# POSTECH-CVLab/InstaOrder

Hardware: AMD Instinct MI355X
Metric: instance-pairs/sec (fwd+bwd) (higher is better)
Workload: dtype f32; 1 GPU; InstaOrderNet_o, pair-batch 256 per GPU at 256x256x5, fp32, fwd+bwd+SGD (BASELINE.json configs[1]); inputs=resident in HBM, pairs_per_gpu=256, input_size=256, parallelism=dp1, hip_graph=True, setup_steps=0, inputs_distinct=True

## Files before the change

### include/instaorder_hip.h

```cpp
#ifndef INSTAORDER_HIP_H
#define INSTAORDER_HIP_H

#include <stddef.h>
#include <stdint.h>

#ifdef __cplusplus
extern "C" {
#endif

#define IO_OK 0
#define IO_ERR_SHAPE (-1)
#define IO_ERR_WORKSPACE (-2)
#define IO_ERR_LAUNCH (-3)
#define IO_ERR_STATE (-4)
#define IO_ERR_NODEVICE (-5)

#if !defined(__HIP__) && !defined(HIP_INCLUDE_HIP_HIP_RUNTIME_API_H)
typedef void* hipStream_t;
#endif

int io_abi_version(void);
const char* io_last_error_string(void);
int io_device_count(void);
int io_set_winograd(int on);
// ... 207 lines not shown
                             const float* scale, const float* shift, float* dgamma, float* dbeta, void* dyb,
                             float* workspace, size_t workspace_floats, int dtype, int gw, hipStream_t stream);
size_t io_stem_packed_floats(int real_channels);
size_t io_stem_wgrad_exact_workspace_bytes(int N, int H, int W, int real_channels);
int io_stem_fwd_bnstats_exact(const float* x8, const float* w, float* y, int N, int H, int W, int real_channels, int G,
                              const float* gamma, const float* beta, float* running_mean, float* running_var,
                              float momentum, float eps, float* mean, float* rstd, float* scale, float* shift,
                              float* workspace, size_t workspace_floats, float* packed, hipStream_t stream);
int io_stem_wgrad_exact(const float* x8, const float* dy, float* dw, int N, int H, int W, int real_channels,
                        void* workspace, size_t workspace_bytes, float* packed, hipStream_t stream);
int io_stem_wgrad_exact_bn(const float* x8, const float* da, const float* y, float* dw, int N, int H, int W,
                           int real_channels, int G, const float* gamma, const float* mean, const float* rstd,
                           const float* scale, const float* shift, float* dgamma, float* dbeta, float* coef,
                           float* bn_partial, size_t bn_partial_floats, void* workspace, size_t workspace_bytes,
                           float* packed, hipStream_t stream);

size_t io_bn_tile_partial_floats(int M, int C, int G);
int io_bn_bwd_coefs_dt(const void* dz, const void* y, int M, int C, int G, const float* gamma, const float* mean,
                       const float* rstd, float* dgamma, float* dbeta, float* coef, float* partial,
                       size_t partial_floats, int dtype, hipStream_t stream);
int io_bn_bwd_coefs_from_tile_partials(float* p1, float* p2, int M, int C, int G, const float* gamma, const float* mean,
                                       const float* rstd, float* dgamma, float* dbeta, float* coef, hipStream_t stream);
typedef struct io_dgrad_fused {
    const void* xb_y;
    const float* xb_coef;
    void* xb_dy_out;
    const void* add;
    const void* relu_mask;
    const void* ep_y;
    const float *ep_mean, *ep_rstd, *ep_scale, *ep_shift;
// ... 159 lines not shown
```

### instaorder_amd/_lib.py

```python
import ctypes as C
import os

_HERE = os.path.dirname(os.path.abspath(__file__))
LIB_PATH = os.environ.get("IO_LIB_PATH") or os.path.join(_HERE, "libinstaorder_hip.so")
_lib = None

c_float_p = C.c_void_p


def csrc_digest():
    import glob
    import hashlib
    h = hashlib.sha256()
    files = sorted(glob.glob(os.path.join(_HERE, "csrc", "*.hip")) + glob.glob(os.path.join(_HERE, "csrc", "*.h")))
    files.append(os.path.join(os.path.dirname(_HERE), "include", "instaorder_hip.h"))
    for f in files:
        h.update(os.path.basename(f).encode())
        h.update(open(f, "rb").read())
    return h.hexdigest()[:16]


class TensorInfo(C.Structure):
    _fields_ = [("name", C.c_char * 64), ("kind", C.c_int), ("ndim", C.c_int), ("shape", C.c_long * 4),
                ("offset", C.c_long), ("numel_storage", C.c_long), ("cin_storage", C.c_int),
# ... 140 lines not shown
    "io_add": (_I, [_P, _P, _Z, _P, _I, _P]),
    "io_colsum_partial_floats": (_Z, [_I, _I]),
    "io_colsum": (_I, [_P, _I, _I, _P, _P, _Z, _I, _P]),
    "io_head1_fwd": (_I, [_P, _I, _I, _I, _P, _P, _I, _P, _I, _P]),
    "io_head1_bwd": (_I, [_P, _P, _P, _I, _I, _I, _P, _I, _P, _P, _P, _P, _Z, _I, _P]),
    "io_conv2d_fwd_bnstats_dt": (_I, [_P, _P, _P, _I, _I, _I, _I, _I, _I, _I, _I, _I, _I, _P, _P, _P, _P, _F, _F, _P,
                                      _P, _P, _P, _P, _Z, _I, _I, _P]),
    "io_conv2d_fwd_bias_dt": (_I, [_P, _P, _P, _I, _I, _I, _I, _I, _I, _I, _I, _I, _P, _P, _I, _I, _I, _P]),
    "io_stem_packed_floats": (_Z, [_I]),
    "io_stem_wgrad_exact_workspace_bytes": (_Z, [_I, _I, _I, _I]),
    "io_stem_fwd_bnstats_exact": (_I, [_P, _P, _P, _I, _I, _I, _I, _I, _P, _P, _P, _P, _F, _F, _P, _P, _P, _P, _P, _Z, _P,
                                       _P]),
    "io_stem_wgrad_exact": (_I, [_P, _P, _P, _I, _I, _I, _I, _P, _Z, _P, _P]),
    "io_stem_wgrad_exact_bn": (_I, [_P, _P, _P, _P, _I, _I, _I, _I, _I, _P, _P, _P, _P, _P, _P, _P, _P, _P, _Z, _P, _Z, _P,
                                    _P]),
    "io_stem_wgrad_bn_bf16": (_I, [_P, _P, _P, _P, _I, _I, _I, _I, _P, _P, _P, _P, _P, _P, _P, _P, _P, _Z, _P, _Z, _P]),
    "io_stem_wgrad_bf16_workspace_bytes": (_Z, []),
    "io_debug_last_wgrad_route": (_I, []),
    "io_conv2d_fwd_resid": (_I, [_P, _P, _P, _P, _P, _I, _I, _I, _I, _I, _I, _P, _P, _P, _P, _P, _P, _P, _F, _F, _P, _P, _P,
                                 _P, _P, _Z, _P]),
    "io_smooth_loss_workspace_floats": (_Z, [_I, _I, _I]),
    "io_smooth_loss_fwd": (_I, [_P, _P, _I, _I, _I, _F, _P, _P, _P, _Z, _P]),
    "io_smooth_loss_bwd": (_I, [_P, _P, _P, _F, _I, _I, _I, _I, _P, _P]),
    "io_disp_order_workspace_floats": (_Z, [_I, _I, _I]),
    "io_disp_order_count": (_I, [_P, _P, _P, _P, _P, _P, _I, _I, _I, _I, _F, _P, _P, _Z, _P]),
    "io_bn_tile_partial_floats": (_Z, [_I, _I, _I]),
    "io_bn_bwd_coefs_dt": (_I, [_P, _P, _I, _I, _I, _P, _P, _P, _P, _P, _P, _P, _Z, _I, _P]),
    "io_bn_bwd_coefs_from_tile_partials": (_I, [_P, _P, _I, _I, _I, _P, _P, _P, _P, _P, _P, _P]),
    "io_conv2d_dgrad_fused_dt": (_I, [_P, _P, _P, _I, _I, _I, _I, _I, _I, _I, _I, _I, C.POINTER(DgradFused), _I, _P]),
    "io_conv2d_dgrad_bnbwd_dt": (_I, [_P, _P, _P, _I, _I, _I, _I, _I, _I, _I, _I, _P, _I, _P, _P, _P, _P, _P, _P, _P, _P, _P,
# ... 62 lines not shown
```

### instaorder_amd/csrc/bn.hip

```cpp
#include "io_common.h"

namespace {

constexpr int kThreads = 256;

template <typename T> __device__ __forceinline__ f32x4 ld4(const T* p) { return io_ldv(p); }
template <typename T> __device__ __forceinline__ void st4(T* p, f32x4 v) { io_stv(p, v); }

__device__ __forceinline__ f32x4 bn_affine(f32x4 y, f32x4 mean, f32x4 scale, f32x4 shift) {
    f32x4 r;
#pragma unroll
    for (int k = 0; k < 4; ++k) r[k] = __builtin_fmaf(y[k] - mean[k], scale[k], shift[k]);
    return r;
}

template <typename T> struct Chunk {
    static constexpr int VEC = 16 / (int)sizeof(T), NV = VEC / 4;
    f32x4 v[NV];
};
__device__ __forceinline__ Chunk<float> ldc(const float* p) {
    Chunk<float> c;
    c.v[0] = *reinterpret_cast<const f32x4*>(p);
    return c;
}
// ... 323 lines not shown
                            }
                            s1[i][k] += dd;
                            s2[i][k] += dd * ((yv[u].v[k] - mu[i].v[k]) * rs[i].v[k]);
                        }
                    }
                }
            }
        }
    }
    const size_t o = ((size_t)g * nb + b) * C;
#pragma unroll
    for (int k = 0; k < NV; ++k) {
        f32x4 t1[2] = {s1[0][k], s1[1][k]}, t2[2] = {s2[0][k], s2[1][k]};
        reduce_rows_store<2>(cm, t1, t2, p1 + o + 4 * k, p2 + o + 4 * k, CV, VEC);
    }
}

__global__ __launch_bounds__(256) void bn_bwd_finalize_kernel(const float* __restrict__ p1,
                                                             const float* __restrict__ p2, int nb, int G, int Mg,
                                                             int C, float* __restrict__ dgamma,
                                                             float* __restrict__ dbeta, float* __restrict__ c1,
                                                             float* __restrict__ c2,
                                                             const float* __restrict__ xgamma = nullptr,
                                                             const float* __restrict__ xmean = nullptr,
                                                             const float* __restrict__ xrstd = nullptr,
                                                             float* __restrict__ c3 = nullptr) {
    constexpr int U = 16;
    __shared__ double sh[2][32][8];
    const int tx = threadIdx.x & 7, ty = threadIdx.x >> 3;
    const int c = blockIdx.x * 8 + tx;
// ... 452 lines not shown
    const int rpb = bn_rows_per_block(Mg, G, &nb);
    float* p1 = partial;
    float* p2 = partial + (size_t)G * nb * C;
    IoProfScope prof(IO_PROF_BN_BWD, 0.0, (double)io_dtype_bytes(dt) * M * C * 2.0, st);
    if (dt == IO_BF16)
        hipLaunchKernelGGL(bn_bwd_reduce_kernel<bf16_t>, dim3(nb, G), dim3(kThreads), 0, st, (const bf16_t*)dz,
                           (const bf16_t*)nullptr, (const bf16_t*)y, Mg, C, rpb, mean, rstd, mask_scale, mask_shift, p1, p2);
    else
        hipLaunchKernelGGL(bn_bwd_reduce_kernel<float>, dim3(nb, G), dim3(kThreads), 0, st, (const float*)dz,
                           (const float*)nullptr, (const float*)y, Mg, C, rpb, mean, rstd, mask_scale, mask_shift, p1, p2);
    hipLaunchKernelGGL(bn_bwd_finalize_kernel, dim3(io_cdiv(C, 8)), dim3(256), 0, st, p1, p2, nb, G, Mg, C, dgamma, dbeta,
                       coef, coef + (size_t)G * C, gamma, mean, rstd, coef + (size_t)2 * G * C);
    return io_check_launch("bn_bwd_coefs");
}

namespace {
__global__ __launch_bounds__(256) void bn_resid2_tables_kernel(const float* __restrict__ m3, const float* __restrict__ s3,
                                                              const float* __restrict__ h3, const float* __restrict__ md,
                                                              const float* __restrict__ sd, const float* __restrict__ hd,
                                                              int n, float* __restrict__ coef) {
    const int i = blockIdx.x * 256 + threadIdx.x;
    if (i >= n) return;
    coef[i] = s3[i];
    coef[n + i] = sd[i];
    coef[2 * n + i] = (float)(((double)h3[i] - (double)m3[i] * (double)s3[i]) + ((double)hd[i] - (double)md[i] * (double)sd[i]));
}
}

int io_bn_resid2_tables(const float* mean3, const float* scale3, const float* shift3, const float* meand,
                        const float* scaled, const float* shiftd, int G, int C, float* coef, hipStream_t st) {
// ... 7 lines not shown
```

### instaorder_amd/csrc/capi.hip

```cpp
#include <stdarg.h>
#include <stdio.h>
#include <stdlib.h>
#include <string.h>

#include "io_common.h"

static thread_local char g_err[512] = "";

void io_set_error(const char* fmt, ...) {
    va_list ap;
    va_start(ap, fmt);
    vsnprintf(g_err, sizeof(g_err), fmt, ap);
    va_end(ap);
}

int io_check_launch(const char* what) {
    hipError_t e = hipGetLastError();
    if (e != hipSuccess) {
        io_set_error("%s: %s", what, hipGetErrorString(e));
        return IO_ERR_LAUNCH;
    }
    return IO_OK;
}

// ... 471 lines not shown
    if (rc) return rc;
    IoStemXb xb{};
    xb.y = y;
    xb.a = coef;
    xb.b = coef + (size_t)G * 64;
    xb.c = coef + (size_t)2 * G * 64;
    xb.mean = mean;
    xb.scale = scale;
    xb.shift = shift;
    xb.G = G;
    rc = io_launch_stem_wgrad_rows(g, x8, da, packed, (float*)ws, ws_bytes, st, &xb);
    if (rc) return rc;
    return io_stem_unpack_grad(packed, dw, 64, 49, real_channels, st);
}

extern "C" size_t io_stem_wgrad_bf16_workspace_bytes(void) { return io_stem_wgrad_halo_partial_bytes(); }
extern "C" int io_stem_wgrad_bn_bf16(const void* x8, const void* da, const void* y, float* dw, int N, int H, int W, int G,
                                     const float* gamma, const float* mean, const float* rstd, const float* scale,
                                     const float* shift, float* dgamma, float* dbeta, float* coef, float* bn_partial,
                                     size_t bn_partial_floats, void* ws, size_t ws_bytes, hipStream_t st) {
    IO_REQUIRE(x8 && da && y && dw && coef && ws, IO_ERR_SHAPE, "stem_wgrad_bn_bf16: null argument");
    IoConvGeom g = io_geom_fwd(N, H, W, 8, 64, 7, 7, 2, 3);
    IO_REQUIRE(io_stem_wgrad_halo_ok(g, ws_bytes, G), IO_ERR_SHAPE,
               "stem_wgrad_bn_bf16: needs 256 x 256 inputs (128-wide output rows), G | N, io_stem_wgrad_bf16_workspace_bytes() of "
               "workspace and enough rows for the persistent blocks (else: io_bn_bwd_dt + io_conv2d_wgrad_dt)");
    const int M = N * g.Ho * g.Wo;
    int rc = io_bn_bwd_coefs_t(da, y, M, 64, G, gamma, mean, rstd, dgamma, dbeta, coef, bn_partial, bn_partial_floats, st, IO_BF16,
                               scale, shift);
    if (rc) return rc;
    IoStemXb xb{};
// ... 186 lines not shown
```

### instaorder_amd/csrc/io_common.h

```cpp
#pragma once
#include <hip/hip_runtime.h>
#include <stdint.h>
#include <stddef.h>

#include "../../include/instaorder_hip.h"

void io_set_error(const char* fmt, ...);
int io_check_launch(const char* what);

#define IO_REQUIRE(cond, code, ...)        \
    do {                                   \
        if (!(cond)) {                     \
            io_set_error(__VA_ARGS__);     \
            return (code);                 \
        }                                  \
    } while (0)

static inline int io_cdiv(long a, long b) { return (int)((a + b - 1) / b); }

#include <atomic>
static inline int io_device_cu_count() {
    static std::atomic<int> cache[64];
    int dev = 0;
    if (hipGetDevice(&dev) != hipSuccess || dev < 0 || dev >= 64) return 256;
// ... 35 lines not shown
__device__ __forceinline__ f32x4 io_ldv(const bf16_t* p) {
    const uint2 r = *reinterpret_cast<const uint2*>(p);
    f32x4 v;
    v[0] = __builtin_bit_cast(float, r.x << 16);
    v[1] = __builtin_bit_cast(float, r.x & 0xffff0000u);
    v[2] = __builtin_bit_cast(float, r.y << 16);
    v[3] = __builtin_bit_cast(float, r.y & 0xffff0000u);
    return v;
}
__device__ __forceinline__ void io_stv(float* p, f32x4 v) { *reinterpret_cast<f32x4*>(p) = v; }
__device__ __forceinline__ void io_stv(bf16_t* p, f32x4 v) {
    uint2 r;
    r.x = io_f2bf2(v[0], v[1]);
    r.y = io_f2bf2(v[2], v[3]);
    *reinterpret_cast<uint2*>(p) = r;
}
#endif

struct IoFastDiv {
    unsigned magic;
    int shift;
};
static inline IoFastDiv io_fastdiv(int d) {
    IoFastDiv f;
    if (d <= 1) { f.magic = 0; f.shift = -1; return f; }
    int s = 0;
    while ((1LL << s) < d) ++s;
    const unsigned long long num = 1ULL << (31 + s);
    f.magic = (unsigned)((num + (unsigned long long)d - 1) / (unsigned long long)d);
    f.shift = s - 1;
// ... 100 lines not shown
int io_bn_finalize_tiles(float* tile_mean, float* tile_m2, int M, int C, int G, const float* gamma,
                         const float* beta, float* running_mean, float* running_var, float momentum, float eps,
                         float* mean, float* rstd, float* scale, float* shift, hipStream_t st);
int io_launch_conv_wgrad(const IoConvGeom& g, const void* in, const void* dy, float* dw, float* partial,
                         size_t partial_bytes, int stem, hipStream_t st, int dt_in = IO_F32, int dt_dy = IO_F32);
size_t io_conv_wgrad_partial_bytes(const IoConvGeom& g, int stem);

IoConvGeom io_geom_fwd(int N, int H, int W, int Cin, int Cout, int R, int S, int stride, int pad);
bool io_stem_rows_ok(const IoConvGeom& g);
int io_launch_stem_rows(const IoConvGeom& g, const float* x8, const float* wp, float* out, float* st_mean, float* st_m2,
                        const float* bias, int relu, hipStream_t st);
int io_stem_wgrad_rows_max_blocks();
struct IoStemXb {
    const float *y, *a, *b, *c, *mean, *scale, *shift;
    int G, tiles_per_group;
};
int io_launch_stem_wgrad_rows(const IoConvGeom& g, const float* x8, const float* dy, float* dwp, float* partial,
                              size_t partial_bytes, hipStream_t st, const IoStemXb* xb = nullptr);
size_t io_stem_wgrad_halo_partial_bytes();
bool io_stem_wgrad_halo_ok(const IoConvGeom& g, size_t partial_bytes, int G);
int io_launch_stem_wgrad_halo(const IoConvGeom& g, const void* x8, const void* dz, float* dw, float* partial, size_t partial_bytes,
                              hipStream_t st, const IoStemXb* xb);
size_t io_wgrad_halo3_partial_bytes();
bool io_wgrad_halo3_shape(const IoConvGeom& g);
int io_launch_conv_wgrad_halo3(const IoConvGeom& g, const void* x, const void* dy, float* dw, float* partial, size_t partial_bytes,
                               hipStream_t st);
int io_splitk_reduce(const float* partial, float* dst, size_t n4, int splits, hipStream_t st);
struct IoFilterTable {
    static constexpr int kMax = 64;
    int n;
    int start[kMax + 1];
// ... 23 lines not shown
```

### instaorder_amd/csrc/net.hip

```cpp
#include <stdio.h>
#include <string.h>

#include <vector>

#include "io_common.h"

namespace {

constexpr int kMaxGroups = 8;
constexpr float kBnEps = 1e-5f, kBnMomentum = 0.1f;

struct ConvL {
    int cin, cout, k, stride, pad, cin_store;
    long w_off;
};
struct BnL {
    int C;
    long g_off, b_off, run_off;
    int index;
};
struct Block {
    ConvL c1, c2, c3, cd;
    BnL b1, b2, b3, bd;
    bool down;
// ... 654 lines not shown
    if (L.stride == 1 && whole_tiles(M, c.G)) {
        IoBwStats bw = bw_for(c, b, y, M, true);
        bw.a_out = a_out;
        if (xb) xb_fill(c, bw, *xb, xb_y, xb_M, xb_out);
        if (c.plan.wino_u != kNoBuf && L.k == 3 && c.dt() == IO_F32 && !xb) bw.wino_u = c.buf(c.plan.wino_u);
        IO_TRY(conv_dgrad(c, L, dy, dx, nullptr, nullptr, H, &bw));
        if (!dyb) return IO_OK;
        return bn_back_tiles(c, b, dx, y, M, dyb);
    }
    IO_REQUIRE(!xb && dyb, IO_ERR_STATE, "dgrad_then_bn: the operand transform needs the fused path");
    IO_REQUIRE(!a_out, IO_ERR_STATE, "dgrad_then_bn: no fused epilogue to rebuild the activation in");
    IO_TRY(conv_dgrad(c, L, dy, dx, nullptr, nullptr, H));
    return bn_back(c, b, dx, 1, nullptr, y, M, dyb, nullptr);
}

int stem_bn_coefs(const Ctx& c, const void* dz, IoStemXb& xb) {
    const BnL& b = c.net->bn1;
    Tables t = c.tables(b);
    IO_TRY(io_bn_bwd_coefs_t(dz, c.act(c.plan.y0), c.N * (c.S / 2) * (c.S / 2), b.C, c.G, c.params + b.g_off, t.mean, t.rstd,
                             c.grads + b.g_off, c.grads + b.b_off, c.buf(c.plan.coef), c.buf(c.plan.bn_partial),
                             c.plan.bn_partial_floats, c.st, c.dt(), t.scale, t.shift));
    const size_t gs = (size_t)c.G * b.C;
    xb = IoStemXb{};
    xb.y = (const float*)c.act(c.plan.y0);
    xb.a = c.buf(c.plan.coef);
    xb.b = c.buf(c.plan.coef) + gs;
    xb.c = c.buf(c.plan.coef) + 2 * gs;
    xb.mean = t.mean;
    xb.scale = t.scale;
    xb.shift = t.shift;
    xb.G = c.G;
    return IO_OK;
}

int run_backward(Ctx& c, const float* dlogits, const void* x8, int stage_lo = 0, int stage_hi = kBwdStages) {
    const io_net* net = c.net;
    const Plan& p = c.plan;
    void* Ga = c.act(p.gbuf[2]);
// ... 56 lines not shown
        }
        if (x1) IO_TRY(bn_back_coefs(c, b.b1, Ga, c.act(bb.y1), Min, x1d));
        {
            IoBwStats bw{};
            const bool carry = r.carry;
            if (carry) bw = bw_for(c, net->blocks[ii - 1].b3, c.act(p.blk[ii - 1].y3), Min, false);
            if (x1) xb_fill(c, bw, b.b1, c.act(bb.y1), Min, Gb);
            const uint32_t* mbits = (ii > 0 && c.routes[ii - 1].bits_written) ? bits_of(c, ii - 1) : nullptr;
            if (mbits) bw.maskbits = mbits;
            IO_TRY(conv_dgrad(c, b.c1, x1 ? Ga : Gb, Ge, partial, xmask, H, (carry || x1 || mbits) ? &bw : nullptr));
        }
        if (x1) IO_TRY(conv_wgrad(c, b.c1, xin, Gb, H));
    }
    if (stage_hi < kBwdStages) return IO_OK;
    void *Gd = dout_buf(-1), *Ge = dout_buf(0);
    IO_TRY(io_maxpool_bwd_t(Gd, reinterpret_cast<const uint32_t*>(c.ws + p.idx0), c.N, H0, H0, 64, Ge, c.st, c.dt()));
    {
        IoConvGeom g = io_geom_fwd(c.N, c.S, c.S, 8, 64, 7, 7, 2, 3);
        g.cr = net->stem.cin;
        if (stem_exact(c, net->stem) && io_stem_rows_ok(g) && c.N % c.G == 0) {
            IoStemXb xb;
            IO_TRY(stem_bn_coefs(c, Ge, xb));
            IO_TRY(io_launch_stem_wgrad_rows(g, (const float*)x8, (const float*)Ge, c.buf(c.plan.stem_dwp),
                                             c.buf(c.plan.wg_partial), c.plan.wg_partial_bytes, c.st, &xb));
            return io_stem_unpack_grad(c.buf(c.plan.stem_dwp), c.grads + net->stem.w_off, net->stem.cout, 49,
                                       net->stem.cin, c.st);
        }
    }
    if (c.net->dtype == IO_BF16) {
        IoConvGeom g = io_geom_fwd(c.N, c.S, c.S, 8, 64, 7, 7, 2, 3);
        if (io_stem_wgrad_halo_ok(g, c.plan.wg_partial_bytes, c.G)) {
            IoStemXb xb;
            IO_TRY(stem_bn_coefs(c, Ge, xb));
            return io_launch_stem_wgrad_halo(g, x8, Ge, c.grads + net->stem.w_off, c.buf(c.plan.wg_partial),
                                             c.plan.wg_partial_bytes, c.st, &xb);
        }
    }
    IO_TRY(bn_back(c, net->bn1, Ge, 1, nullptr, c.act(p.y0), c.N * H0 * H0, Ga, nullptr));
    IO_TRY(conv_wgrad(c, net->stem, x8, Ga, c.S));
    return IO_OK;
}

}
// ... 216 lines not shown
```

### instaorder_amd/csrc/stem.hip

```cpp
#include <hip/hip_runtime.h>

#include <type_traits>

#include "io_common.h"

#ifndef IO_STEM_ABLATE
#define IO_STEM_ABLATE 0
#endif

typedef float f32x2 __attribute__((ext_vector_type(2)));
typedef float f32x4 __attribute__((ext_vector_type(4)));
typedef float f32x16 __attribute__((ext_vector_type(16)));

namespace {
constexpr int kCR = 5;
constexpr int kPW = 262;
constexpr int kPitch = kPW * kCR;
constexpr int kKB = 36;
constexpr int kBImg = 7 * 64 * kKB;
constexpr int kPix = 7 * kPW;
constexpr int kNT = 512;
constexpr int kRounds = (kPix + kNT - 1) / kNT;
constexpr int kPatch = kRounds * kNT * kCR;
constexpr int kRed = 2 * 4 * 64 * 2;
// ... 144 lines not shown
        __syncthreads();
        pacc = acc;
        cur ^= 1;
    };
    for (int t = t_lo; t <= t_hi + 1; ++t) {
        if (t > t_lo + 1 && t + 1 < t_hi) body(std::true_type{}, t);
        else body(std::false_type{}, t);
    }
}

constexpr int kWPitch = 1315;
constexpr int kWPatch = kRounds * kNT * kCR + 40;
constexpr int kWDy = 128 * 64;
constexpr size_t kWLds = (size_t)2 * (kWPatch + kWDy) * sizeof(float);

template <bool XB>
__global__ __launch_bounds__(kNT, 1) void stem_wgrad_rows_kernel(const float* __restrict__ x8, const float* __restrict__ dy,
                                                                 float* __restrict__ partial, int Hi, int Wi, int Ho, int Wo,
                                                                 int ntiles, int per_block, IoStemXb xb) {
    extern __shared__ __attribute__((aligned(16))) float smem[];
    float* sP = smem;
    float* sD = smem + 2 * kWPatch;
    const int tid = threadIdx.x, lane = tid & 63, wave = tid >> 6;
    const int l32 = lane & 31, h = lane >> 5;
    const int t_lo = blockIdx.x * per_block, t_hi = min(ntiles, t_lo + per_block);
    const int cbn = Wo >> 7;

    float pr[kRounds][kCR];
    f32x4 dr[4], yr[4], tb[6];
    int p_r[kRounds], p_c[kRounds], p_off[kRounds], p_dst[kRounds];
    bool p_ok[kRounds];
#pragma unroll
    for (int i = 0; i < kRounds; ++i) {
        const int p = tid + i * kNT;
        p_r[i] = p / kPW;
        p_c[i] = p - p_r[i] * kPW;
        p_off[i] = (p_r[i] * Wi + p_c[i]) * 8;
        p_dst[i] = p_r[i] * kWPitch + p_c[i] * kCR;
        if (p >= kPix || p_c[i] >= kPW - 1) p_r[i] = 1 << 20;
    }
    int f_cb = t_lo % cbn, f_ho = (t_lo / cbn) % Ho, f_n = (t_lo / cbn) / Ho;
    const float* f_dy = dy + (size_t)t_lo * kWDy + tid * 4;
    const float* f_y = XB ? xb.y + (size_t)t_lo * kWDy + tid * 4 : nullptr;
    int f_t = t_lo;
    auto fetch = [&]() {
        const int hi0 = 2 * f_ho - 3, wi0 = 256 * f_cb - 3;
        const float* base = x8 + (((ptrdiff_t)f_n * Hi + hi0) * Wi + wi0) * 8;
        if (++f_cb == cbn) {
            f_cb = 0;
            if (++f_ho == Ho) {
                f_ho = 0;
                ++f_n;
            }
        }
#pragma unroll
        for (int i = 0; i < kRounds; ++i) {
            const bool ok = (unsigned)(hi0 + p_r[i]) < (unsigned)Hi && (unsigned)(wi0 + p_c[i]) < (unsigned)Wi;
            const float* src = ok ? base + p_off[i] : x8;
            const f32x4 v = *reinterpret_cast<const f32x4*>(src);
            pr[i][0] = v.x; pr[i][1] = v.y; pr[i][2] = v.z; pr[i][3] = v.w;
            pr[i][4] = src[4];
            p_ok[i] = ok;
        }
#pragma unroll
        for (int i = 0; i < 4; ++i) dr[i] = *reinterpret_cast<const f32x4*>(f_dy + i * kNT * 4);
        f_dy += kWDy;
        if constexpr (XB) {
#pragma unroll
            for (int i = 0; i < 4; ++i) yr[i] = *reinterpret_cast<const f32x4*>(f_y + i * kNT * 4);
            f_y += kWDy;
            const int go = (f_t / xb.tiles_per_group) * 64 + (tid & 15) * 4;
            ++f_t;
            tb[0] = *reinterpret_cast<const f32x4*>(xb.a + go);
            tb[1] = *reinterpret_cast<const f32x4*>(xb.b + go);
            tb[2] = *reinterpret_cast<const f32x4*>(xb.c + go);
            tb[3] = *reinterpret_cast<const f32x4*>(xb.mean + go);
            tb[4] = *reinterpret_cast<const f32x4*>(xb.scale + go);
            tb[5] = *reinterpret_cast<const f32x4*>(xb.shift + go);
        }
    };
    auto stage = [&](int buf) {
        float* dst = sP + buf * kWPatch;
#pragma unroll
        for (int i = 0; i < kRounds; ++i)
#pragma unroll
            for (int c = 0; c < kCR; ++c) dst[p_dst[i] + c] = p_ok[i] ? pr[i][c] : 0.f;
        float* dd = sD + buf * kWDy + tid * 4;
#pragma unroll
        for (int i = 0; i < 4; ++i) {
            f32x4 v = dr[i];
            if constexpr (XB) {
#pragma unroll
                for (int e = 0; e < 4; ++e) {
                    const float act = __builtin_fmaf(yr[i][e] - tb[3][e], tb[4][e], tb[5][e]);
                    const float dz = act > 0.f ? v[e] : 0.f;
                    v[e] = __builtin_fmaf(tb[0][e], dz, __builtin_fmaf(tb[1][e], yr[i][e], tb[2][e]));
                }
            }
            *reinterpret_cast<f32x4*>(dd + i * kNT * 4) = v;
        }
    };

    fetch();
    stage(0);
    __syncthreads();

    const int j = wave * 32 + l32;
    const int jr = min(j, 7 * 7 * kCR - 1) / (7 * kCR), jk = min(j, 7 * 7 * kCR - 1) - jr * 7 * kCR;
    const int b_lane = jr * kWPitch + jk + 2 * kCR * h;
    const int a_lane = h * 64 + l32;
    f32x16 acc0, acc1;
#pragma unroll
    for (int r = 0; r < 16; ++r) acc0[r] = acc1[r] = 0.f;
    int cur = 0;
    auto mma_tile = [&]() {
        const float* pb = sP + cur * kWPatch + b_lane;
        const float* pa = sD + cur * kWDy + a_lane;
        float fb[2][8], fa0[2][8], fa1[2][8];
        auto read_chunk = [&](int c, int s) {
#pragma unroll
            for (int i = 0; i < 8; ++i) {
                fb[s][i] = pb[(c * 8 + i) * 4 * kCR];
                fa0[s][i] = pa[(c * 8 + i) * 128];
                fa1[s][i] = pa[(c * 8 + i) * 128 + 32];
            }
        };
        read_chunk(0, 0);
#pragma unroll
        for (int c = 0; c < 8; ++c) {
            if (c + 1 < 8) read_chunk(c + 1, (c + 1) & 1);
#pragma unroll
            for (int i = 0; i < 8; ++i) {
                acc0 = __builtin_amdgcn_mfma_f32_32x32x2f32(fa0[c & 1][i], fb[c & 1][i], acc0, 0, 0, 0);
                acc1 = __builtin_amdgcn_mfma_f32_32x32x2f32(fa1[c & 1][i], fb[c & 1][i], acc1, 0, 0, 0);
            }
            __builtin_amdgcn_sched_barrier(0);
        }
    };
    for (int t = t_lo; t < t_hi; ++t) {
        if (t + 1 < t_hi) {
            fetch();
            __builtin_amdgcn_sched_barrier(0);
            mma_tile();
            stage(cur ^ 1);
        } else {
            mma_tile();
        }
        __syncthreads();
        cur ^= 1;
    }
    float* o = partial + ((size_t)blockIdx.x * 64 + 4 * h) * 256 + j;
    const bool real = j < 7 * 7 * kCR;
#pragma unroll
    for (int r = 0; r < 16; ++r) {
        const int row = (r & 3) + 8 * (r >> 2);
        o[(size_t)row * 256] = real ? acc0[r] : 0.f;
        o[(size_t)(row + 32) * 256] = real ? acc1[r] : 0.f;
    }
}
}

// ... 21 lines not shown
    const int ncu = ncu_of[dev & 63] > 0 ? ncu_of[dev & 63] : 256;
    const int blocks = ntiles < ncu ? ntiles : ncu;
    const int per_block = (ntiles + blocks - 1) / blocks;
    const dim3 grid((unsigned)((ntiles + per_block - 1) / per_block));
    if (st_mean)
        hipLaunchKernelGGL(stem_rows_kernel<true>, grid, dim3(kNT), kLds, st, x8, wp, io_stem_kp(g.wT, g.cr), out, st_mean,
                           st_m2, bias, relu, g.Hi, g.Wi, g.Ho, g.Wo, ntiles, per_block);
    else
        hipLaunchKernelGGL(stem_rows_kernel<false>, grid, dim3(kNT), kLds, st, x8, wp, io_stem_kp(g.wT, g.cr), out, st_mean,
                           st_m2, bias, relu, g.Hi, g.Wi, g.Ho, g.Wo, ntiles, per_block);
    return io_check_launch("stem_rows");
}

int io_stem_wgrad_rows_max_blocks() { return 256; }

int io_launch_stem_wgrad_rows(const IoConvGeom& g, const float* x8, const float* dy, float* dwp, float* partial,
                              size_t partial_bytes, hipStream_t st, const IoStemXb* xb) {
    IO_REQUIRE(io_stem_rows_ok(g), IO_ERR_SHAPE, "stem_wgrad_rows: not the 7x7 stride-2 stem on whole 128-pixel output rows");
    const int ntiles = g.N * g.Ho * (g.Wo / 128);
    static std::atomic<unsigned long long> seen{0};
    static int ncu_of[64];
    int dev = 0;
    if (io_first_on_device(seen, &dev)) {
        hipDeviceProp_t prop;
        int n = hipGetDeviceProperties(&prop, dev) == hipSuccess ? prop.multiProcessorCount : 0;
        ncu_of[dev & 63] = (n <= 0 || n > io_stem_wgrad_rows_max_blocks()) ? io_stem_wgrad_rows_max_blocks() : n;
        (void)hipFuncSetAttribute((const void*)stem_wgrad_rows_kernel<false>, hipFuncAttributeMaxDynamicSharedMemorySize, (int)kWLds);
        (void)hipFuncSetAttribute((const void*)stem_wgrad_rows_kernel<true>, hipFuncAttributeMaxDynamicSharedMemorySize, (int)kWLds);
    }
    const int ncu = ncu_of[dev & 63] > 0 ? ncu_of[dev & 63] : io_stem_wgrad_rows_max_blocks();
    const int blocks = ntiles < ncu ? ntiles : ncu;
    const int per_block = (ntiles + blocks - 1) / blocks;
    const int grid = (ntiles + per_block - 1) / per_block;
    IO_REQUIRE(partial && partial_bytes >= (size_t)grid * 64 * 256 * sizeof(float), IO_ERR_WORKSPACE,
               "stem_wgrad_rows: workspace %zu < %zu bytes", partial_bytes, (size_t)grid * 64 * 256 * sizeof(float));
    IoStemXb x{};
    if (xb) {
        x = *xb;
        IO_REQUIRE(x.y && x.a && x.b && x.c && x.mean && x.scale && x.shift && x.G >= 1 && g.N % x.G == 0, IO_ERR_SHAPE,
                   "stem_wgrad_rows: the fused BatchNorm backward needs y, six [G][64] tables and G | N");
        x.tiles_per_group = ntiles / x.G;
    }
    const double Md = (double)g.N * g.Ho * g.Wo;
    {
        IoProfScope prof(IO_PROF_WGRAD_STEM, 2.0 * Md * 64 * 49.0 * kCR,
                         4.0 * (Md * 64 * (xb ? 2.0 : 1.0) + (double)g.N * g.Hi * g.Wi * 8 + 64.0 * 49 * kCR), st);
        if (xb)
            hipLaunchKernelGGL(stem_wgrad_rows_kernel<true>, dim3((unsigned)grid), dim3(kNT), kWLds, st, x8, dy, partial, g.Hi,
                               g.Wi, g.Ho, g.Wo, ntiles, per_block, x);
        else
            hipLaunchKernelGGL(stem_wgrad_rows_kernel<false>, dim3((unsigned)grid), dim3(kNT), kWLds, st, x8, dy, partial, g.Hi,
                               g.Wi, g.Ho, g.Wo, ntiles, per_block, x);
        const int rc = io_check_launch("stem_wgrad_rows");
        if (rc) return rc;
        return io_splitk_reduce(partial, dwp, (size_t)64 * 256 / 4, grid, st);
    }
}
```

Before: 1824 pairs/s.

## Fuse maxpool backward into stem BatchNorm-coef reduction and stem wgrad kernel

Removes the separate maxpool backward pass that wrote a full-resolution gradient for the stem output. The BatchNorm backward reduction and the stem weight-gradient kernel now read the pooled gradient plus the packed tap indices and rebuild each pixel's gradient on the fly. In the wgrad kernel the LDS staging of the next tile is interleaved into the MFMA loop. This saves a full-resolution write and two reads, in exchange for more gather logic, extra registers and possible scheduling pressure in the MFMA kernel. It is enabled by default and can be turned off with an environment variable.

```diff
diff --git a/include/instaorder_hip.h b/include/instaorder_hip.h
--- a/include/instaorder_hip.h
+++ b/include/instaorder_hip.h
@@ -245,6 +245,13 @@
                            const float* scale, const float* shift, float* dgamma, float* dbeta, float* coef,
                            float* bn_partial, size_t bn_partial_floats, void* workspace, size_t workspace_bytes,
                            float* packed, hipStream_t stream);
+int io_stem_wgrad_exact_bn_pooled(const float* x8, const float* dpool, const uint32_t* idx, const float* y, float* dw,
+                                  float* dgamma, float* dbeta, int N, int H, int W, int real_channels, int G,
+                                  const float* gamma, const float* mean, const float* rstd, const float* scale,
+                                  const float* shift, float* coef, void* workspace, size_t workspace_bytes, float* packed,
+                                  hipStream_t stream);
+int io_set_stem_pooled_bwd(int on);
+int io_get_stem_pooled_bwd(void);
 
 size_t io_bn_tile_partial_floats(int M, int C, int G);
 int io_bn_bwd_coefs_dt(const void* dz, const void* y, int M, int C, int G, const float* gamma, const float* mean,
diff --git a/instaorder_amd/_lib.py b/instaorder_amd/_lib.py
--- a/instaorder_amd/_lib.py
+++ b/instaorder_amd/_lib.py
@@ -178,6 +178,10 @@
     "io_stem_wgrad_exact": (_I, [_P, _P, _P, _I, _I, _I, _I, _P, _Z, _P, _P]),
     "io_stem_wgrad_exact_bn": (_I, [_P, _P, _P, _P, _I, _I, _I, _I, _I, _P, _P, _P, _P, _P, _P, _P, _P, _P, _Z, _P, _Z, _P,
                                     _P]),
+    "io_stem_wgrad_exact_bn_pooled": (_I, [_P, _P, _P, _P, _P, _P, _P, _I, _I, _I, _I, _I, _P, _P, _P, _P, _P, _P, _P, _Z, _P,
+                                           _P]),
+    "io_set_stem_pooled_bwd": (_I, [_I]),
+    "io_get_stem_pooled_bwd": (_I, []),
     "io_stem_wgrad_bn_bf16": (_I, [_P, _P, _P, _P, _I, _I, _I, _I, _P, _P, _P, _P, _P, _P, _P, _P, _P, _Z, _P, _Z, _P]),
     "io_stem_wgrad_bf16_workspace_bytes": (_Z, []),
     "io_debug_last_wgrad_route": (_I, []),
diff --git a/instaorder_amd/csrc/bn.hip b/instaorder_amd/csrc/bn.hip
--- a/instaorder_amd/csrc/bn.hip
+++ b/instaorder_amd/csrc/bn.hip
@@ -361,6 +361,88 @@
         f32x4 t1[2] = {s1[0][k], s1[1][k]}, t2[2] = {s2[0][k], s2[1][k]};
         reduce_rows_store<2>(cm, t1, t2, p1 + o + 4 * k, p2 + o + 4 * k, CV, VEC);
     }
+}
+
+template <typename T>
+__global__ __launch_bounds__(kThreads) void stem_pool_bn_reduce_kernel(const T* __restrict__ y, const T* __restrict__ dpool,
+                                                                      const uint32_t* __restrict__ idx, int Mg, int H,
+                                                                      int W, int rpb, int w_shift, int h_shift,
+                                                                      const float* __restrict__ mean,
+                                                                      const float* __restrict__ rstd,
+                                                                      const float* __restrict__ mscale,
+                                                                      const float* __restrict__ mshift,
+                                                                      float* __restrict__ p1, float* __restrict__ p2) {
+    static_assert(sizeof(T) == 4, "fp32 storage only");
+    constexpr int C = 64, CV = C / 4, U = 4;
+    const ColMap cm = col_map(CV);
+    const int g = blockIdx.y, b = blockIdx.x, nb = gridDim.x;
+    const int r0 = b * rpb, r1 = min(r0 + rpb, Mg);
+    const int Hp = (H + 1) / 2, Wp = (W + 1) / 2;
+    const int q = cm.tx;
+    const f32x4 mu = *reinterpret_cast<const f32x4*>(mean + g * C + q * 4);
+    const f32x4 rs = *reinterpret_cast<const f32x4*>(rstd + g * C + q * 4);
+    const f32x4 msc = *reinterpret_cast<const f32x4*>(mscale + g * C + q * 4);
+    const f32x4 msh = *reinterpret_cast<const f32x4*>(mshift + g * C + q * 4);
+    f32x4 s1[1], s2[1];
+    s1[0] = 0.f; s2[0] = 0.f;
+    for (int r = r0 + cm.ty; r < r1; r += U * cm.TY) {
+        f32x4 yv[U], gv[U][4];
+        uint32_t id[U][4], tap[U];
+        bool two[U];
+#pragma unroll
+        for (int u = 0; u < U; ++u) {
+            const int rr = r + u * cm.TY;
+            if (rr < r1) {
+                const unsigned px = (unsigned)g * (unsigned)Mg + (unsigned)rr;
+                const unsigned row = w_shift >= 0 ? px >> w_shift : px / (unsigned)W;
+                const int w = (int)(px - row * (unsigned)W);
+                const unsigned n = h_shift >= 0 ? row >> h_shift : row / (unsigned)H;
+                const int h = (int)(row - n * (unsigned)H);
+                yv[u] = *reinterpret_cast<const f32x4*>(y + (size_t)px * C + q * 4);
+                const int ho0 = h >> 1, wo0 = w >> 1;
+                const bool ow = (w & 1) && wo0 + 1 < Wp;
+                two[u] = (h & 1) && ho0 + 1 < Hp;
+                tap[u] = (uint32_t)((1 + (h & 1)) * 3 + 1 + (w & 1));
+                const size_t o0 = (((size_t)n * Hp + ho0) * Wp + wo0) * CV + q;
+                id[u][0] = idx[o0];
+                gv[u][0] = *reinterpret_cast<const f32x4*>(dpool + o0 * 4);
+                id[u][1] = id[u][3] = 0xffffffffu;
+                gv[u][1] = gv[u][3] = 0.f;
+                if (ow) {
+                    id[u][1] = idx[o0 + CV];
+                    gv[u][1] = *reinterpret_cast<const f32x4*>(dpool + (o0 + CV) * 4);
+                }
+                if (two[u]) {
+                    const size_t o2 = o0 + (size_t)Wp * CV;
+                    id[u][2] = idx[o2];
+                    gv[u][2] = *reinterpret_cast<const f32x4*>(dpool + o2 * 4);
+                    if (ow) {
+                        id[u][3] = idx[o2 + CV];
+                        gv[u][3] = *reinterpret_cast<const f32x4*>(dpool + (o2 + CV) * 4);
+                    }
+                }
+            }
+        }
+#pragma unroll
+        for (int u = 0; u < U; ++u) {
+            if (r + u * cm.TY < r1) {
+                f32x4 da = 0.f;
+                io_pool_tap_add(da, id[u][0], gv[u][0], tap[u]);
+                io_pool_tap_add(da, id[u][1], gv[u][1], tap[u] - 2);
+                if (two[u]) {
+                    io_pool_tap_add(da, id[u][2], gv[u][2], tap[u] - 6);
+                    io_pool_tap_add(da, id[u][3], gv[u][3], 0);
+                }
+                const f32x4 av = bn_affine(yv[u], mu, msc, msh);
+#pragma unroll
+                for (int e = 0; e < 4; ++e) da[e] = av[e] > 0.f ? da[e] : 0.f;
+                s1[0] += da;
+                s2[0] += da * ((yv[u] - mu) * rs);
+            }
+        }
+    }
+    const size_t o = ((size_t)g * nb + b) * C;
+    reduce_rows_store<1>(cm, s1, s2, p1 + o, p2 + o, CV, 4);
 }
 
 __global__ __launch_bounds__(256) void bn_bwd_finalize_kernel(const float* __restrict__ p1,
@@ -843,6 +925,28 @@
     return io_check_launch("bn_bwd_coefs");
 }
 
+int io_stem_pool_bn_coefs(const float* y, const float* dpool, const uint32_t* idx, int N, int H, int W, int G,
+                          const float* gamma, const float* mean, const float* rstd, const float* scale, const float* shift,
+                          float* dgamma, float* dbeta, float* coef, float* partial, size_t partial_floats, hipStream_t st) {
+    constexpr int C = 64;
+    IO_REQUIRE(y && dpool && idx && scale && shift && coef, IO_ERR_SHAPE, "stem_pool_bn_coefs: null argument");
+    IO_REQUIRE(N > 0 && H > 0 && W > 0 && G >= 1 && N % G == 0 && (double)N * H * W < 2.0e9, IO_ERR_SHAPE,
+               "stem_pool_bn_coefs: N=%d H=%d W=%d must be positive, below 2^31 pixels, and N divisible by G=%d", N, H, W, G);
+    const int M = N * H * W, Mg = M / G;
+    IO_REQUIRE(partial_floats >= io_bn_partial_floats(M, C, G), IO_ERR_WORKSPACE, "stem_pool_bn_coefs: partial too small");
+    int nb;
+    const int rpb = bn_rows_per_block(Mg, G, &nb);
+    float* p1 = partial;
+    float* p2 = partial + (size_t)G * nb * C;
+    const double Mp = (double)N * ((H + 1) / 2) * ((W + 1) / 2);
+    IoProfScope prof(IO_PROF_BN_BWD, 0.0, 4.0 * M * C + Mp * C * (4.0 + 1.0), st);
+    hipLaunchKernelGGL(stem_pool_bn_reduce_kernel<float>, dim3(nb, G), dim3(kThreads), 0, st, y, dpool, idx, Mg, H, W, rpb,
+                       ilog2_exact(W), ilog2_exact(H), mean, rstd, scale, shift, p1, p2);
+    hipLaunchKernelGGL(bn_bwd_finalize_kernel, dim3(io_cdiv(C, 8)), dim3(256), 0, st, p1, p2, nb, G, Mg, C, dgamma, dbeta,
+                       coef, coef + (size_t)G * C, gamma, mean, rstd, coef + (size_t)2 * G * C);
+    return io_check_launch("stem_pool_bn_coefs");
+}
+
 namespace {
 __global__ __launch_bounds__(256) void bn_resid2_tables_kernel(const float* __restrict__ m3, const float* __restrict__ s3,
                                                               const float* __restrict__ h3, const float* __restrict__ md,
diff --git a/instaorder_amd/csrc/capi.hip b/instaorder_amd/csrc/capi.hip
--- a/instaorder_amd/csrc/capi.hip
+++ b/instaorder_amd/csrc/capi.hip
@@ -509,6 +509,40 @@
     return io_stem_unpack_grad(packed, dw, 64, 49, real_channels, st);
 }
 
+extern "C" int io_stem_wgrad_exact_bn_pooled(const float* x8, const float* dpool, const uint32_t* idx, const float* y, float* dw,
+                                             float* dgamma, float* dbeta, int N, int H, int W, int real_channels, int G,
+                                             const float* gamma, const float* mean, const float* rstd, const float* scale,
+                                             const float* shift, float* coef, void* ws, size_t ws_bytes, float* packed,
+                                             hipStream_t st) {
+    IO_REQUIRE(real_channels >= 1 && real_channels <= 8 && packed && coef, IO_ERR_SHAPE,
+               "stem_wgrad_exact_bn_pooled: real_channels=%d (1..8)", real_channels);
+    IO_REQUIRE(x8 && dpool && idx && y && dw && dgamma && dbeta && gamma && mean && rstd && scale && shift, IO_ERR_SHAPE,
+               "stem_wgrad_exact_bn_pooled: null argument (idx: the pooling forward's tap words)");
+    IoConvGeom g = stem_geom_exact(N, H, W, real_channels);
+    IO_REQUIRE(io_stem_rows_ok(g) && G >= 1 && N % G == 0, IO_ERR_SHAPE,
+               "stem_wgrad_exact_bn_pooled: needs 5 real channels, 256 | H, W and G | N (else: io_maxpool_bwd + io_bn_bwd + "
+               "io_stem_wgrad_exact)");
+    const size_t bn_floats = io_bn_partial_floats(N * g.Ho * g.Wo, 64, G);
+    const size_t need = std::max(bn_floats * sizeof(float), io_conv_wgrad_partial_bytes(g, 1));
+    IO_REQUIRE(ws && ws_bytes >= need, IO_ERR_WORKSPACE, "stem_wgrad_exact_bn_pooled: workspace %zu < %zu bytes", ws_bytes, need);
+    int rc = io_stem_pool_bn_coefs(y, dpool, idx, N, g.Ho, g.Wo, G, gamma, mean, rstd, scale, shift, dgamma, dbeta, coef, (float*)ws,
+                                   bn_floats, st);
+    if (rc) return rc;
+    IoStemXb xb{};
+    xb.y = y;
+    xb.a = coef;
+    xb.b = coef + (size_t)G * 64;
+    xb.c = coef + (size_t)2 * G * 64;
+    xb.mean = mean;
+    xb.scale = scale;
+    xb.shift = shift;
+    xb.G = G;
+    xb.idx = idx;
+    rc = io_launch_stem_wgrad_rows(g, x8, dpool, packed, (float*)ws, ws_bytes, st, &xb);
+    if (rc) return rc;
+    return io_stem_unpack_grad(packed, dw, 64, 49, real_channels, st);
+}
+
 extern "C" size_t io_stem_wgrad_bf16_workspace_bytes(void) { return io_stem_wgrad_halo_partial_bytes(); }
 extern "C" int io_stem_wgrad_bn_bf16(const void* x8, const void* da, const void* y, float* dw, int N, int H, int W, int G,
                                      const float* gamma, const float* mean, const float* rstd, const float* scale,
diff --git a/instaorder_amd/csrc/io_common.h b/instaorder_amd/csrc/io_common.h
--- a/instaorder_amd/csrc/io_common.h
+++ b/instaorder_amd/csrc/io_common.h
@@ -73,6 +73,11 @@
     r.x = io_f2bf2(v[0], v[1]);
     r.y = io_f2bf2(v[2], v[3]);
     *reinterpret_cast<uint2*>(p) = r;
+}
+__device__ __forceinline__ void io_pool_tap_add(f32x4& acc, uint32_t id, f32x4 g, uint32_t tap) {
+#pragma unroll
+    for (int e = 0; e < 4; ++e)
+        if (((id >> (8 * e)) & 0xffu) == tap) acc[e] += g[e];
 }
 #endif
 
@@ -203,7 +208,12 @@
 struct IoStemXb {
     const float *y, *a, *b, *c, *mean, *scale, *shift;
     int G, tiles_per_group;
-};
+    const uint32_t* idx;
+};
+int io_stem_pooled_bwd_enabled();
+int io_stem_pool_bn_coefs(const float* y, const float* dpool, const uint32_t* idx, int N, int H, int W, int G,
+                          const float* gamma, const float* mean, const float* rstd, const float* scale, const float* shift,
+                          float* dgamma, float* dbeta, float* coef, float* partial, size_t partial_floats, hipStream_t st);
 int io_launch_stem_wgrad_rows(const IoConvGeom& g, const float* x8, const float* dy, float* dwp, float* partial,
                               size_t partial_bytes, hipStream_t st, const IoStemXb* xb = nullptr);
 size_t io_stem_wgrad_halo_partial_bytes();
diff --git a/instaorder_amd/csrc/net.hip b/instaorder_amd/csrc/net.hip
--- a/instaorder_amd/csrc/net.hip
+++ b/instaorder_amd/csrc/net.hip
@@ -692,14 +692,20 @@
     return bn_back(c, b, dx, 1, nullptr, y, M, dyb, nullptr);
 }
 
-int stem_bn_coefs(const Ctx& c, const void* dz, IoStemXb& xb) {
+int stem_bn_coefs(const Ctx& c, const void* dz, IoStemXb& xb, const float* dpool = nullptr, const uint32_t* idx = nullptr) {
     const BnL& b = c.net->bn1;
     Tables t = c.tables(b);
-    IO_TRY(io_bn_bwd_coefs_t(dz, c.act(c.plan.y0), c.N * (c.S / 2) * (c.S / 2), b.C, c.G, c.params + b.g_off, t.mean, t.rstd,
-                             c.grads + b.g_off, c.grads + b.b_off, c.buf(c.plan.coef), c.buf(c.plan.bn_partial),
-                             c.plan.bn_partial_floats, c.st, c.dt(), t.scale, t.shift));
+    if (idx)
+        IO_TRY(io_stem_pool_bn_coefs((const float*)c.act(c.plan.y0), dpool, idx, c.N, c.S / 2, c.S / 2, c.G, c.params + b.g_off,
+                                     t.mean, t.rstd, t.scale, t.shift, c.grads + b.g_off, c.grads + b.b_off,
+                                     c.buf(c.plan.coef), c.buf(c.plan.bn_partial), c.plan.bn_partial_floats, c.st));
+    else
+        IO_TRY(io_bn_bwd_coefs_t(dz, c.act(c.plan.y0), c.N * (c.S / 2) * (c.S / 2), b.C, c.G, c.params + b.g_off, t.mean,
+                                 t.rstd, c.grads + b.g_off, c.grads + b.b_off, c.buf(c.plan.coef), c.buf(c.plan.bn_partial),
+                                 c.plan.bn_partial_floats, c.st, c.dt(), t.scale, t.shift));
     const size_t gs = (size_t)c.G * b.C;
     xb = IoStemXb{};
+    xb.idx = idx;
     xb.y = (const float*)c.act(c.plan.y0);
     xb.a = c.buf(c.plan.coef);
     xb.b = c.buf(c.plan.coef) + gs;
@@ -786,19 +792,26 @@
     }
     if (stage_hi < kBwdStages) return IO_OK;
     void *Gd = dout_buf(-1), *Ge = dout_buf(0);
-    IO_TRY(io_maxpool_bwd_t(Gd, reinterpret_cast<const uint32_t*>(c.ws + p.idx0), c.N, H0, H0, 64, Ge, c.st, c.dt()));
+    const uint32_t* idx0 = reinterpret_cast<const uint32_t*>(c.ws + p.idx0);
     {
         IoConvGeom g = io_geom_fwd(c.N, c.S, c.S, 8, 64, 7, 7, 2, 3);
         g.cr = net->stem.cin;
         if (stem_exact(c, net->stem) && io_stem_rows_ok(g) && c.N % c.G == 0) {
+            const bool pooled = io_stem_pooled_bwd_enabled() != 0;
             IoStemXb xb;
-            IO_TRY(stem_bn_coefs(c, Ge, xb));
-            IO_TRY(io_launch_stem_wgrad_rows(g, (const float*)x8, (const float*)Ge, c.buf(c.plan.stem_dwp),
+            if (pooled) {
+                IO_TRY(stem_bn_coefs(c, nullptr, xb, (const float*)Gd, idx0));
+            } else {
+                IO_TRY(io_maxpool_bwd_t(Gd, idx0, c.N, H0, H0, 64, Ge, c.st, c.dt()));
+                IO_TRY(stem_bn_coefs(c, Ge, xb));
+            }
+            IO_TRY(io_launch_stem_wgrad_rows(g, (const float*)x8, (const float*)(pooled ? Gd : Ge), c.buf(c.plan.stem_dwp),
                                              c.buf(c.plan.wg_partial), c.plan.wg_partial_bytes, c.st, &xb));
             return io_stem_unpack_grad(c.buf(c.plan.stem_dwp), c.grads + net->stem.w_off, net->stem.cout, 49,
                                        net->stem.cin, c.st);
         }
     }
+    IO_TRY(io_maxpool_bwd_t(Gd, idx0, c.N, H0, H0, 64, Ge, c.st, c.dt()));
     if (c.net->dtype == IO_BF16) {
         IoConvGeom g = io_geom_fwd(c.N, c.S, c.S, 8, 64, 7, 7, 2, 3);
         if (io_stem_wgrad_halo_ok(g, c.plan.wg_partial_bytes, c.G)) {
diff --git a/instaorder_amd/csrc/stem.hip b/instaorder_amd/csrc/stem.hip
--- a/instaorder_amd/csrc/stem.hip
+++ b/instaorder_amd/csrc/stem.hip
@@ -182,7 +182,7 @@
 constexpr int kWDy = 128 * 64;
 constexpr size_t kWLds = (size_t)2 * (kWPatch + kWDy) * sizeof(float);
 
-template <bool XB>
+template <bool XB, bool POOL>
 __global__ __launch_bounds__(kNT, 1) void stem_wgrad_rows_kernel(const float* __restrict__ x8, const float* __restrict__ dy,
                                                                  float* __restrict__ partial, int Hi, int Wi, int Ho, int Wo,
                                                                  int ntiles, int per_block, IoStemXb xb) {
@@ -195,7 +195,18 @@
     const int cbn = Wo >> 7;
 
     float pr[kRounds][kCR];
+    static_assert(XB || !POOL, "the pooled form rides on the BatchNorm form");
     f32x4 dr[4], yr[4], tb[6];
+    f32x4 ga[4], gb[4];
+    uint32_t ia[4], ib[4];
+    uint32_t f_kh = 1;
+    const int pm = tid >> 4;
+    auto slot = [&](int i) { return POOL ? tid * 4 + (pm + (i & 1) + 64 * (i >> 1)) * 64 : tid * 4 + i * kNT * 4; };
+    const int Hp = (Ho + 1) >> 1, Wp = (Wo + 1) >> 1;
+    int p_lo[4];
+#pragma unroll
+    for (int j = 0; j < 4; ++j) p_lo[j] = (pm + (j & 1) + 32 * (j >> 1)) * 16 + (tid & 15);
+    const bool p_past = pm == 31;
     int p_r[kRounds], p_c[kRounds], p_off[kRounds], p_dst[kRounds];
     bool p_ok[kRounds];
 #pragma unroll
@@ -209,11 +220,12 @@
     }
     int f_cb = t_lo % cbn, f_ho = (t_lo / cbn) % Ho, f_n = (t_lo / cbn) / Ho;
     const float* f_dy = dy + (size_t)t_lo * kWDy + tid * 4;
-    const float* f_y = XB ? xb.y + (size_t)t_lo * kWDy + tid * 4 : nullptr;
+    const float* f_y = XB ? xb.y + (size_t)t_lo * kWDy : nullptr;
     int f_t = t_lo;
     auto fetch = [&]() {
         const int hi0 = 2 * f_ho - 3, wi0 = 256 * f_cb - 3;
         const float* base = x8 + (((ptrdiff_t)f_n * Hi + hi0) * Wi + wi0) * 8;
+        const int c_n = f_n, c_ho = f_ho, c_cb = f_cb;
         if (++f_cb == cbn) {
             f_cb = 0;
             if (++f_ho == Ho) {
@@ -230,12 +242,48 @@
             pr[i][4] = src[4];
             p_ok[i] = ok;
         }
-#pragma unroll
-        for (int i = 0; i < 4; ++i) dr[i] = *reinterpret_cast<const f32x4*>(f_dy + i * kNT * 4);
-        f_dy += kWDy;
+        if constexpr (POOL) {
+            const int hp0 = c_ho >> 1;
+            const bool two = (c_ho & 1) && hp0 + 1 < Hp;
+            f_kh = 1 + (c_ho & 1);
+            const size_t ra = (((size_t)c_n * Hp + hp0) * Wp + 64 * c_cb) * 16;
+            const float* ga_row = dy + ra * 4;
+            const uint32_t* ia_row = xb.idx + ra;
+            const bool past = p_past && c_cb == cbn - 1;
+            const int o3 = past ? p_lo[3] - 16 : p_lo[3];
+            const uint32_t off3 = past ? 0xffffffffu : 0u;
+#pragma unroll
+            for (int j = 0; j < 4; ++j) {
+                const int o = j == 3 ? o3 : p_lo[j];
+                ia[j] = ia_row[o];
+                ga[j] = *reinterpret_cast<const f32x4*>(ga_row + o * 4);
+            }
+            ia[3] |= off3;
+            if (two) {
+                const float* gb_row = ga_row + (size_t)Wp * 64;
+                const uint32_t* ib_row = ia_row + (size_t)Wp * 16;
+#pragma unroll
+                for (int j = 0; j < 4; ++j) {
+                    const int o = j == 3 ? o3 : p_lo[j];
+                    ib[j] = ib_row[o];
+                    gb[j] = *reinterpret_cast<const f32x4*>(gb_row + o * 4);
+                }
+                ib[3] |= off3;
+            } else {
+#pragma unroll
+                for (int j = 0; j < 4; ++j) {
+                    ib[j] = 0xffffffffu;
+                    gb[j] = 0.f;
+                }
+            }
+        } else {
+#pragma unroll
+            for (int i = 0; i < 4; ++i) dr[i] = *reinterpret_cast<const f32x4*>(f_dy + i * kNT * 4);
+            f_dy += kWDy;
+        }
         if constexpr (XB) {
 #pragma unroll
-            for (int i = 0; i < 4; ++i) yr[i] = *reinterpret_cast<const f32x4*>(f_y + i * kNT * 4);
+            for (int i = 0; i < 4; ++i) yr[i] = *reinterpret_cast<const f32x4*>(f_y + slot(i));
             f_y += kWDy;
             const int go = (f_t / xb.tiles_per_group) * 64 + (tid & 15) * 4;
             ++f_t;
@@ -247,16 +295,26 @@
             tb[5] = *reinterpret_cast<const f32x4*>(xb.shift + go);
         }
     };
-    auto stage = [&](int buf) {
+    auto stage_part = [&](int buf, int i) {
         float* dst = sP + buf * kWPatch;
 #pragma unroll
-        for (int i = 0; i < kRounds; ++i)
-#pragma unroll
-            for (int c = 0; c < kCR; ++c) dst[p_dst[i] + c] = p_ok[i] ? pr[i][c] : 0.f;
-        float* dd = sD + buf * kWDy + tid * 4;
-#pragma unroll
-        for (int i = 0; i < 4; ++i) {
-            f32x4 v = dr[i];
+        for (int c = 0; c < kCR; ++c) dst[p_dst[i] + c] = p_ok[i] ? pr[i][c] : 0.f;
+        float* dd = sD + buf * kWDy;
+        {
+            f32x4 v = 0.f;
+            if constexpr (!POOL) v = dr[i];
+            if constexpr (POOL) {
+                const int j = 2 * (i >> 1);
+                if (i & 1) {
+                    io_pool_tap_add(v, ia[j], ga[j], f_kh * 3 + 2);
+                    io_pool_tap_add(v, ia[j + 1], ga[j + 1], f_kh * 3);
+                    io_pool_tap_add(v, ib[j], gb[j], 2);
+                    io_pool_tap_add(v, ib[j + 1], gb[j + 1], 0);
+                } else {
+                    io_pool_tap_add(v, ia[j], ga[j], f_kh * 3 + 1);
+                    io_pool_tap_add(v, ib[j], gb[j], 1);
+                }
+            }
             if constexpr (XB) {
 #pragma unroll
                 for (int e = 0; e < 4; ++e) {
@@ -265,8 +323,12 @@
                     v[e] = __builtin_fmaf(tb[0][e], dz, __builtin_fmaf(tb[1][e], yr[i][e], tb[2][e]));
                 }
             }
-            *reinterpret_cast<f32x4*>(dd + i * kNT * 4) = v;
-        }
+            *reinterpret_cast<f32x4*>(dd + slot(i)) = v;
+        }
+    };
+    auto stage = [&](int buf) {
+#pragma unroll
+        for (int i = 0; i < 4; ++i) stage_part(buf, i);
     };
 
     fetch();
@@ -281,7 +343,8 @@
 #pragma unroll
     for (int r = 0; r < 16; ++r) acc0[r] = acc1[r] = 0.f;
     int cur = 0;
-    auto mma_tile = [&]() {
+    auto mma_tile = [&](auto staged) {
+        constexpr bool INLINE = POOL && decltype(staged)::value;
         const float* pb = sP + cur * kWPatch + b_lane;
         const float* pa = sD + cur * kWDy + a_lane;
         float fb[2][8], fa0[2][8], fa1[2][8];
@@ -302,6 +365,8 @@
                 acc0 = __builtin_amdgcn_mfma_f32_32x32x2f32(fa0[c & 1][i], fb[c & 1][i], acc0, 0, 0, 0);
                 acc1 = __builtin_amdgcn_mfma_f32_32x32x2f32(fa1[c & 1][i], fb[c & 1][i], acc1, 0, 0, 0);
             }
+            if constexpr (INLINE)
+                if (c >= 4) stage_part(cur ^ 1, c - 4);
             __builtin_amdgcn_sched_barrier(0);
         }
     };
@@ -309,10 +374,10 @@
         if (t + 1 < t_hi) {
             fetch();
             __builtin_amdgcn_sched_barrier(0);
-            mma_tile();
-            stage(cur ^ 1);
+            mma_tile(std::true_type{});
+            if constexpr (!POOL) stage(cur ^ 1);
         } else {
-            mma_tile();
+            mma_tile(std::false_type{});
         }
         __syncthreads();
         cur ^= 1;
@@ -364,6 +429,24 @@
 
 int io_stem_wgrad_rows_max_blocks() { return 256; }
 
+
+static std::atomic<int> g_stem_pooled{-1};
+int io_stem_pooled_bwd_enabled() {
+    int on = g_stem_pooled.load(std::memory_order_relaxed);
+    if (on < 0) {
+        const char* e = getenv("IO_STEM_POOLED_BWD");
+        on = (e && e[0] == '0') ? 0 : 1;
+        g_stem_pooled.store(on, std::memory_order_relaxed);
+    }
+    return on;
+}
+extern "C" int io_get_stem_pooled_bwd(void) { return io_stem_pooled_bwd_enabled(); }
+extern "C" int io_set_stem_pooled_bwd(int on) {
+    const int prev = io_stem_pooled_bwd_enabled();
+    g_stem_pooled.store(on ? 1 : 0, std::memory_order_relaxed);
+    return prev;
+}
+
 int io_launch_stem_wgrad_rows(const IoConvGeom& g, const float* x8, const float* dy, float* dwp, float* partial,
                               size_t partial_bytes, hipStream_t st, const IoStemXb* xb) {
     IO_REQUIRE(io_stem_rows_ok(g), IO_ERR_SHAPE, "stem_wgrad_rows: not the 7x7 stride-2 stem on whole 128-pixel output rows");
@@ -375,8 +458,9 @@
         hipDeviceProp_t prop;
         int n = hipGetDeviceProperties(&prop, dev) == hipSuccess ? prop.multiProcessorCount : 0;
         ncu_of[dev & 63] = (n <= 0 || n > io_stem_wgrad_rows_max_blocks()) ? io_stem_wgrad_rows_max_blocks() : n;
-        (void)hipFuncSetAttribute((const void*)stem_wgrad_rows_kernel<false>, hipFuncAttributeMaxDynamicSharedMemorySize, (int)kWLds);
-        (void)hipFuncSetAttribute((const void*)stem_wgrad_rows_kernel<true>, hipFuncAttributeMaxDynamicSharedMemorySize, (int)kWLds);
+        (void)hipFuncSetAttribute((const void*)stem_wgrad_rows_kernel<false, false>, hipFuncAttributeMaxDynamicSharedMemorySize, (int)kWLds);
+        (void)hipFuncSetAttribute((const void*)stem_wgrad_rows_kernel<true, false>, hipFuncAttributeMaxDynamicSharedMemorySize, (int)kWLds);
+        (void)hipFuncSetAttribute((const void*)stem_wgrad_rows_kernel<true, true>, hipFuncAttributeMaxDynamicSharedMemorySize, (int)kWLds);
     }
     const int ncu = ncu_of[dev & 63] > 0 ? ncu_of[dev & 63] : io_stem_wgrad_rows_max_blocks();
     const int blocks = ntiles < ncu ? ntiles : ncu;
@@ -393,13 +477,17 @@
     }
     const double Md = (double)g.N * g.Ho * g.Wo;
     {
+        const double dy_floats = (xb && x.idx) ? (Md / 4) * (64 + 16) : Md * 64;
         IoProfScope prof(IO_PROF_WGRAD_STEM, 2.0 * Md * 64 * 49.0 * kCR,
-                         4.0 * (Md * 64 * (xb ? 2.0 : 1.0) + (double)g.N * g.Hi * g.Wi * 8 + 64.0 * 49 * kCR), st);
-        if (xb)
-            hipLaunchKernelGGL(stem_wgrad_rows_kernel<true>, dim3((unsigned)grid), dim3(kNT), kWLds, st, x8, dy, partial, g.Hi,
+                         4.0 * (dy_floats + (xb ? Md * 64 : 0.0) + (double)g.N * g.Hi * g.Wi * 8 + 64.0 * 49 * kCR), st);
+        if (xb && x.idx)
+            hipLaunchKernelGGL((stem_wgrad_rows_kernel<true, true>), dim3((unsigned)grid), dim3(kNT), kWLds, st, x8, dy, partial,
+                               g.Hi, g.Wi, g.Ho, g.Wo, ntiles, per_block, x);
+        else if (xb)
+            hipLaunchKernelGGL((stem_wgrad_rows_kernel<true, false>), dim3((unsigned)grid), dim3(kNT), kWLds, st, x8, dy, partial, g.Hi,
                                g.Wi, g.Ho, g.Wo, ntiles, per_block, x);
         else
-            hipLaunchKernelGGL(stem_wgrad_rows_kernel<false>, dim3((unsigned)grid), dim3(kNT), kWLds, st, x8, dy, partial, g.Hi,
+            hipLaunchKernelGGL((stem_wgrad_rows_kernel<false, false>), dim3((unsigned)grid), dim3(kNT), kWLds, st, x8, dy, partial, g.Hi,
                                g.Wi, g.Ho, g.Wo, ntiles, per_block, x);
         const int rc = io_check_launch("stem_wgrad_rows");
         if (rc) return rc;
```

Result: no change. 1831 pairs/s, median of 6 (+0.4%).
